# sebcossu/yocto_raytracing

Measured on AMD Instinct MI355X. Metric: Mrays/sec + ms/frame, instance10000 1920×1080×64spp, 1/2/4/8 MI355X, higher is better.
Workload: dtype f32; 1 GPU; instance10000 1920x1080 8x8 spp, amb 0.1, one frame per step; scene=instance10000, width=1920, height=1080, spp=64, parallelism=single GPU, algorithm=wavefront

## Files before the change

### yocto_raytracing_amd/csrc/packet_trace.h

```cpp
#pragma once

#include "descent_asm.h"
#include "fast_div.h"
#include "wide_asm.h"
#include "trace_common.h"

namespace yrt {

__device__ __forceinline__ int uniform(int x) { return __builtin_amdgcn_readfirstlane(x); }
__device__ __forceinline__ int lane_now() {
    int l;
    asm volatile("v_mbcnt_lo_u32_b32 %0, -1, 0\n v_mbcnt_hi_u32_b32 %0, -1, %0" : "=v"(l));
    return l;
}
__device__ __forceinline__ unsigned long long ballot(bool p) { return __ballot(p); }
extern "C" __device__ int yrt_llvm_writelane(int value, int lane, int old) __asm("llvm.amdgcn.writelane.i32");
__device__ __forceinline__ int writelane(int old, int value, int lane) { return yrt_llvm_writelane(value, lane, old); }

typedef int sgpr4 __attribute__((ext_vector_type(4)));
typedef int sgpr8 __attribute__((ext_vector_type(8)));
typedef int sgpr16 __attribute__((ext_vector_type(16)));
template <typename V>
__device__ __forceinline__ float4 rec_of(const V& v, int k) {
    return {__int_as_float(v[4 * k]), __int_as_float(v[4 * k + 1]), __int_as_float(v[4 * k + 2]),
// ... 629 lines not shown
                inst_next = lstart;
                inst_end = lstart + lcount;
                avail = lmask;
                if (LM) {
                    const uint32_t skip = (lcl >> 16) & 0x7fffu;
                    if (skip) {
                        const uint32_t keep = ~skip & ((1u << lcount) - 1u);
                        if (!keep) {
                            inst_end = inst_next;
                        } else {
                            inst_next = lstart + __builtin_ctz(keep);
                            inst_end = lstart + 32 - __builtin_clz(keep);
                        }
                    }
                }
                level = 1;
                base = sp;
            } else {
                const bool in = lane_in(lmask);
                unsigned long long leaf_hits = 0;
                DBG_CHECK(lstart >= 0 && lstart + lcount <= S.nsprims, 2, lstart, lcount, level, kind, sp);
#ifdef YRT_WIDE_STATS
                if (!COUNT) wc.box++, wc.prim += (unsigned)lcount;
#endif
                if (kind == kind_triangles) {
                    for (int i = lstart; i < lstart + lcount; i++) {
                        float4 pv[3];
                        ld_records_at<3>(S.sprims, (unsigned)(3 * i), pv);
                        if (COUNT && in) wc.prim++;
                        if (COUNT && (me & 1)) wc.wprim++;
                        float t, w1, w2;
                        const unsigned long long hm =
                            tri_hit_mask<true>(co, cd, tmin, tmax, xyz(pv[0]), xyz(pv[1]), xyz(pv[2]), t, w1, w2, lmask);
                        if (hm) {
                            const bool h = lane_in(hm);
                            tmax = h ? t : tmax;
                            hslot = h ? cur_slot : hslot;
                            hei = h ? ibits(pv[0].w) : hei;
                            hw1 = h ? w1 : hw1;
                            hw2 = h ? w2 : hw2;
                            leaf_hits |= hm;
                        }
                    }
                } else {
                    for (int i = lstart; i < lstart + lcount; i++) {
                        float4 pv[3];
                        ld_records_at<3>(S.sprims, (unsigned)(3 * i), pv);
                        if (COUNT && in) wc.prim++;
                        if (COUNT && (me & 1)) wc.wprim++;
                        float t;
                        vec4f ew;
                        const ray3 lr = {co, cd, tmin, tmax};
                        bool h = kind == kind_lines ? line_hit(lr, xyz(pv[0]), xyz(pv[1]), pv[1].w, pv[2].x, t, ew)
                                                    : point_hit(lr, xyz(pv[0]), pv[1].x, t, ew);
                        h = h && in;
                        tmax = h ? t : tmax;
                        hslot = h ? cur_slot : hslot;
                        hei = h ? ibits(pv[0].w) : hei;
                        hw1 = h ? ew.y : hw1;
                        hw2 = h ? ew.z : hw2;
                        leaf_hits |= ballot(h);
                    }
                }
                done |= leaf_hits & ballot(is_nan(tmax));
                avail &= ~done;
            }
        }
        bool finished = false;
        for (;;) {
            if (level == 1 && sp == base) {
                if (inst_next < inst_end) {
                    const int k = inst_next++;
                    DBG_CHECK(k >= 0 && k < S.ninst, 3, k, inst_end, sp, base, 0);
#ifdef YRT_WIDE_STATS
                    if (!COUNT) wc.inst++;
#endif
                    float4 fr[4];
                    ld_records_at<4>(S.tinst, (unsigned)(4 * k), fr);
                    const frame3f f = {xyz(fr[0]), xyz(fr[1]), xyz(fr[2]), xyz(fr[3])};
                    co = transform_point_inverse(f, wo);
                    const bool ident = (uniform(ibits(fr[0].w)) & (int)inst_identity_bit) != 0;
                    if (ident)
                        cd = icd, ci = ici;
                    else
                        enter_direction(f, wd, live & ~done, cd, ci);
                    const uint32_t rk = (uint32_t)uniform(ibits(fr[3].w));
                    pbase = S.spair + spine_record_f4 * (rk & 0x3fffffffu);
                    kind = (int)(rk >> 30);
                    cur_slot = k;
                    mask = avail;
                    if (COUNT && (mask & me)) wc.inst++;
                    node = 0;
                    oct = ident ? ioct : wave_octant(ci, live & ~done);
                    if (mask) break;
                    continue;
                }
                level = 0;
                avail = live & ~done;
                pbase = ptop;
                co = wo;
                cd = wd;
                {
                    const int t = wave * 64 + lane_now();
                    ci = {wi_lds[0][t], wi_lds[1][t], wi_lds[2][t]};
                }
                oct = woct;
            }
            if (sp == 0) {
                finished = true;
                break;
            }
            if constexpr (SM) {
                sp--;
                node = __builtin_amdgcn_readlane(stk_node, sp);
                mask = ((unsigned long long)(uint32_t)__builtin_amdgcn_readlane(stk_mhi, sp) << 32 |
                        (uint32_t)__builtin_amdgcn_readlane(stk_mlo, sp)) &
                       ~done;
                if (mask) break;
            } else {
                mask = avail;
                if (!mask) {
                    sp = level ? base : 0;
                    continue;
                }
                sp--;
                node = __builtin_amdgcn_readlane(stk_node, sp);
                break;
            }
        }
        if (finished) {
            if (!LM) break;
            lstep = true;
        }
    }
#ifdef YRT_WIDE_STATS
    if (!COUNT) {
        const unsigned long long hitl = ballot(hslot >= 0) & live;
        if ((threadIdx.x & 63) == 0) {
            unsigned long long* line = g_first_stats + 16 * ((blockIdx.x * 7u + threadIdx.x / 64u) & 1023u);
            const unsigned long long v[10] = {1, wc.tex, wc.wnode, wc.inst, wc.wprim, wc.box, wc.prim, 0,
                                              (unsigned long long)__popcll(live), (unsigned long long)__popcll(hitl)};
            for (int i = 0; i < 10; i++) atomicAdd(line + i, v[i]);
        }
        wc = work_counts{};
    }
#endif
    if (hslot < 0) return false;
    hr.slot = hslot;
    hr.ei = hei;
    hr.ew = {1 - hw1 - hw2, hw1, hw2, 0};
    hr.dist = tmax;
    return true;
}

__device__ __forceinline__ void ld_wide_record(const f4* wbase, uint32_t off, float4 (&r)[7]) {
    sgpr16 a;
    sgpr8 b;
    sgpr4 c;
    asm volatile(
        "s_load_dwordx16 %0, %3, %4\n s_load_dwordx8 %1, %3, %4 offset:0x40\n s_load_dwordx4 %2, %3, %4 offset:0x60\n"
        " s_waitcnt lgkmcnt(0)"
        : "=&s"(a), "=&s"(b), "=&s"(c)
        : "s"(wbase), "s"(uniform((int)off)));
#pragma unroll
    for (int k = 0; k < 4; k++) r[k] = rec_of(a, k);
    r[4] = rec_of(b, 0), r[5] = rec_of(b, 1), r[6] = rec_of(c, 0);
}

template <int OCT>
__device__ __forceinline__ void wide_tests(const float4 (&r)[7], vec3f co, vec3f ci, float tmin, float tmax,
                                           unsigned long long mask, uint32_t (&w)[4], unsigned long long (&m)[4]) {
    const float lx[4] = {r[0].x, r[0].y, r[0].z, r[0].w}, ly[4] = {r[1].x, r[1].y, r[1].z, r[1].w},
                lz[4] = {r[2].x, r[2].y, r[2].z, r[2].w}, hx[4] = {r[3].x, r[3].y, r[3].z, r[3].w},
                hy[4] = {r[4].x, r[4].y, r[4].z, r[4].w}, hz[4] = {r[5].x, r[5].y, r[5].z, r[5].w};
    w[0] = (uint32_t)uniform(ibits(r[6].x)), w[1] = (uint32_t)uniform(ibits(r[6].y));
    w[2] = (uint32_t)uniform(ibits(r[6].z)), w[3] = (uint32_t)uniform(ibits(r[6].w));
#pragma unroll
    for (int k = 0; k < 4; k++) {
        if (k < 2 || w[k] != wide_leaf) {
            m[k] = ballot(box_oct<OCT>(co, ci, tmin, tmax, lx[k], ly[k], lz[k], hx[k], hy[k], hz[k])) & mask;
        } else
            m[k] = 0;
    }
}

template <int OCT>
__device__ __forceinline__ bool wide_step(const float4 (&r)[7], vec3f co, vec3f ci, float tmin, float tmax,
                                          uint32_t& cur, unsigned long long& mask, int& sp, int& stk_word,
                                          int& stk_mlo, int& stk_mhi, int floor, unsigned long long done) {
    uint32_t w[4];
    unsigned long long m[4];
    wide_tests<OCT>(r, co, ci, tmin, tmax, mask, w, m);
    unsigned long long cm = 0;
    uint32_t cw = 0;
    {
        uint32_t ow;
        unsigned long long om;
        sp = uniform(sp);
        asm volatile(
            "s_cmp_lg_u64 %[m3], 0\n"
            "s_cbranch_scc1 .Lyb32_%=\n"
            "s_cmp_lg_u64 %[m2], 0\n"
            "s_cbranch_scc1 .Lyb21_%=\n"
            "s_cmp_lg_u64 %[m1], 0\n"
            "s_cbranch_scc1 .Lyb10_%=\n"
            "s_cmp_lg_u64 %[m0], 0\n"
            "s_cbranch_scc1 .Lyfin0_%=\n"
            "s_mov_b64 %[cm], 0\n"
            "s_mov_b32 %[cw], 0\n"
            "s_branch .Lyend_%=\n"
            ".Lyb32_%=:\n"
            "s_cmp_lg_u64 %[m2], 0\n"
            "s_cbranch_scc0 .Lyb31_%=\n"
            "s_mov_b32 m0, %[sp]\n"
            "v_writelane_b32 %[sw], %[w3], m0\n"
            "v_writelane_b32 %[sl], %[l3], m0\n"
            "v_writelane_b32 %[sh], %[h3], m0\n"
            "s_add_u32 %[sp], %[sp], 1\n"
            "s_branch .Lyb21_%=\n"
            ".Lyb31_%=:\n"
            "s_cmp_lg_u64 %[m1], 0\n"
            "s_cbranch_scc0 .Lyb30_%=\n"
            "s_mov_b32 m0, %[sp]\n"
            "v_writelane_b32 %[sw], %[w3], m0\n"
            "v_writelane_b32 %[sl], %[l3], m0\n"
            "v_writelane_b32 %[sh], %[h3], m0\n"
            "s_add_u32 %[sp], %[sp], 1\n"
            "s_branch .Lyb10_%=\n"
            ".Lyb30_%=:\n"
            "s_cmp_lg_u64 %[m0], 0\n"
            "s_cbranch_scc0 .Lyfin3_%=\n"
            "s_mov_b32 m0, %[sp]\n"
            "v_writelane_b32 %[sw], %[w3], m0\n"
            "v_writelane_b32 %[sl], %[l3], m0\n"
            "v_writelane_b32 %[sh], %[h3], m0\n"
            "s_add_u32 %[sp], %[sp], 1\n"
            "s_branch .Lyfin0_%=\n"
            ".Lyb21_%=:\n"
            "s_cmp_lg_u64 %[m1], 0\n"
            "s_cbranch_scc0 .Lyb20_%=\n"
            "s_mov_b32 m0, %[sp]\n"
            "v_writelane_b32 %[sw], %[w2], m0\n"
            "v_writelane_b32 %[sl], %[l2], m0\n"
            "v_writelane_b32 %[sh], %[h2], m0\n"
            "s_add_u32 %[sp], %[sp], 1\n"
            "s_branch .Lyb10_%=\n"
            ".Lyb20_%=:\n"
            "s_cmp_lg_u64 %[m0], 0\n"
            "s_cbranch_scc0 .Lyfin2_%=\n"
            "s_mov_b32 m0, %[sp]\n"
            "v_writelane_b32 %[sw], %[w2], m0\n"
            "v_writelane_b32 %[sl], %[l2], m0\n"
            "v_writelane_b32 %[sh], %[h2], m0\n"
            "s_add_u32 %[sp], %[sp], 1\n"
            "s_branch .Lyfin0_%=\n"
            ".Lyb10_%=:\n"
            "s_cmp_lg_u64 %[m0], 0\n"
            "s_cbranch_scc0 .Lyfin1_%=\n"
            "s_mov_b32 m0, %[sp]\n"
            "v_writelane_b32 %[sw], %[w1], m0\n"
            "v_writelane_b32 %[sl], %[l1], m0\n"
            "v_writelane_b32 %[sh], %[h1], m0\n"
            "s_add_u32 %[sp], %[sp], 1\n"
            "s_branch .Lyfin0_%=\n"
            ".Lyfin3_%=:\n"
            "s_mov_b32 %[cw], %[w3]\n"
            "s_mov_b64 %[cm], %[m3]\n"
            "s_branch .Lyend_%=\n"
            ".Lyfin2_%=:\n"
            "s_mov_b32 %[cw], %[w2]\n"
            "s_mov_b64 %[cm], %[m2]\n"
            "s_branch .Lyend_%=\n"
            ".Lyfin1_%=:\n"
            "s_mov_b32 %[cw], %[w1]\n"
            "s_mov_b64 %[cm], %[m1]\n"
            "s_branch .Lyend_%=\n"
            ".Lyfin0_%=:\n"
            "s_mov_b32 %[cw], %[w0]\n"
            "s_mov_b64 %[cm], %[m0]\n"
            ".Lyend_%=:\n"
            : [cw] "=&s"(ow), [cm] "=&s"(om), [sp] "+s"(sp), [sw] "+v"(stk_word), [sl] "+v"(stk_mlo),
              [sh] "+v"(stk_mhi)
            : [w0] "s"(w[0]), [w1] "s"(w[1]), [w2] "s"(w[2]), [w3] "s"(w[3]), [m0] "s"(m[0]), [m1] "s"(m[1]),
              [m2] "s"(m[2]), [m3] "s"(m[3]), [l0] "s"((uint32_t)m[0]), [l1] "s"((uint32_t)m[1]),
              [l2] "s"((uint32_t)m[2]), [l3] "s"((uint32_t)m[3]), [h0] "s"((uint32_t)(m[0] >> 32)),
              [h1] "s"((uint32_t)(m[1] >> 32)), [h2] "s"((uint32_t)(m[2] >> 32)), [h3] "s"((uint32_t)(m[3] >> 32))
            : "m0", "scc");
        sp = uniform(sp);
        cw = (uint32_t)uniform((int)ow);
        cm = (unsigned long long)(uint32_t)uniform((int)(om >> 32)) << 32 | (uint32_t)uniform((int)(uint32_t)om);
    }
    mask = cm;
    cur = cw;
    if (cm) return !(cw & wide_leaf);
    {
        int n = 0;
        if (inner_pop(floor, done, n, mask, sp, stk_word, stk_mlo, stk_mhi)) {
            cur = (uint32_t)n;
            return !(cur & wide_leaf);
        }
    }
    return false;
}

template <int OCT, int LDSN, bool ASM = false>
__device__ __forceinline__ void wide_descend(const f4* base, const float4* lds, vec3f co, vec3f ci,
// ... 203 lines not shown
```

### yocto_raytracing_amd/csrc/wavefront.hip

```cpp
#include <hip/hip_runtime.h>

#include <algorithm>
#include <cstdio>
#include <cstdlib>
#include <cstring>
#include <stdexcept>
#include <type_traits>

#include "item_magic.h"
#include "packet_trace.h"
#include "trace_common.h"
#include "yrt_render.h"

namespace yrt {
namespace {

constexpr int WF_BLOCK = 256;
#ifndef YRT_PRIMARY_BLOCK
#define YRT_PRIMARY_BLOCK 64
#endif
#ifndef YRT_SHADOW_BLOCK
#define YRT_SHADOW_BLOCK 64
#endif
template <bool PACKET>
// ... 238 lines not shown
template <bool ANY, bool COUNT, bool PACKET, typename SE>
__device__ __forceinline__ tracer<ANY, COUNT, PACKET, SE> make_tracer(traversal_lds<PACKET, SE>& L) {
    tracer<ANY, COUNT, PACKET, SE> t;
    if constexpr (PACKET)
        t.lane_stk = nullptr;
    else
        t.lane_stk = L.lane + threadIdx.x;
    return t;
}

template <unsigned C>
__device__ __forceinline__ unsigned xcd_runs(unsigned b, unsigned n) {
    constexpr unsigned G = 8u * C;
    if (b >= n / G * G) return b;
    const unsigned w = b % G;
    return b - w + (w % 8u) * C + w / 8u;
}

#ifndef YRT_SHADOW_LIGHT_MINOR
#define YRT_SHADOW_LIGHT_MINOR 24
#endif
#ifndef YRT_XCD_CHUNK_PRIMARY
#define YRT_XCD_CHUNK_PRIMARY 256
#endif

__device__ __forceinline__ vec3f div3(vec3f ke, float rr) {
    if (!__ballot(!(div_nr_ok(ke.x, rr) && div_nr_ok(ke.y, rr) && div_nr_ok(ke.z, rr)))) {
        const float y = rcp_nr(rr);
        return {div_nr(ke.x, rr, y), div_nr(ke.y, rr, y), div_nr(ke.z, rr, y)};
    }
    return ke / rr;
}

__device__ __forceinline__ bool light_term_zero(int info, vec3f nrm, vec3f p, vec3f ro, vec3f l, float r, vec3f ke) {
    const int cls = (info >> 26) & 15;
    const float sd = smax(0.0f, dot(nrm, l));
    const bool first = info >= 0 && cls != 0 && (info & 3) != kind_lines && sd == 0.0f;
    if (!ballot(first)) return false;
    vec3f v, h, ker;
    float vlen, hlen;
    normalize_len(ro - p, v, vlen);
    normalize_len(v + l, h, hlen);
    ker = div3(ke, r * r);
    const float x = smax(0.0f, dot(nrm, h));
    const bool ker_ok = fabsf(ker.x) < 0x1p100f && fabsf(ker.y) < 0x1p100f && fabsf(ker.z) < 0x1p100f;
    const bool ls_zero =
        cls == 1 ? x >= 0.0f && x <= 1.0f
                 : x == 0.0f || (x >= 0x1p-126f && x < 1.0f &&
                                 (float)(16 << ((cls - 2) & 15)) * __builtin_amdgcn_logf(x) < -151.0f);
    return first && ker_ok && ls_zero;
}

__device__ __forceinline__ ray3 camera_ray_w(const dev_camera& cam, int W, int H, int ns, int i, int j, int ii,
                                             int jj, bool in_range = false) {
    const float fns = (float)ns, fw = (float)W, fh = (float)H;
    const float a = ii + 0.5f, b = jj + 0.5f;
    float u, v;
    if (in_range || !__ballot(!(div_nr_ok(a, fns) && div_nr_ok(b, fns)))) {
        const float y = rcp_nr(fns);
        u = i + div_nr(a, fns, y), v = j + div_nr(b, fns, y);
    } else {
        u = i + a / fns, v = j + b / fns;
    }
    if (in_range || !__ballot(!(div_nr_ok(u, fw) && div_nr_ok(v, fh)))) {
        u = div_nr(u, fw, rcp_nr(fw)), v = div_nr(v, fh, rcp_nr(fh));
    } else {
        u = u / fw, v = v / fh;
    }
    vec3f q;
    q.x = cam.ox + (u - 0.5f) * cam.w * cam.xx + (v - 0.5f) * cam.h * cam.yx - cam.focus * cam.zx;
    q.y = cam.oy + (u - 0.5f) * cam.w * cam.xy + (v - 0.5f) * cam.h * cam.yy - cam.focus * cam.zy;
    q.z = cam.oz + (u - 0.5f) * cam.w * cam.xz + (v - 0.5f) * cam.h * cam.yz - cam.focus * cam.zz;
    const vec3f o = {cam.ox, cam.oy, cam.oz};
    vec3f d;
    float len;
    normalize_len(q - o, d, len);
    return {o, d, ray_eps, flt_max};
}

#ifndef YRT_BUNDLE_ITEMS
#define YRT_BUNDLE_ITEMS 64
#endif
constexpr int bundle_g = YRT_BUNDLE_ITEMS;
static_assert(bundle_g >= 1 && bundle_g <= 64, "one item per lane of k_bundle_lists");
#ifndef YRT_BUNDLE_MIN_TOP
#define YRT_BUNDLE_MIN_TOP 8
#endif
#ifndef YRT_LISTS_MIN_SPP
#define YRT_LISTS_MIN_SPP 9
#endif
constexpr int bundle_max = 16;
constexpr int bundle_recs = 5;
constexpr int bundle_max_lights = 8;
#ifndef YRT_CAMERA_LIST_MAX
#define YRT_CAMERA_LIST_MAX 32
#endif
constexpr int camera_list_max = YRT_CAMERA_LIST_MAX;

template <int CTRL, int ROWS>
__device__ __forceinline__ int dpp_i(int v) {
    return __builtin_amdgcn_mov_dpp(v, CTRL, ROWS, 0xf, false);
}
__device__ __forceinline__ int fkey(int b) { return b ^ ((b >> 31) & 0x7fffffff); }
template <bool MAX>
__device__ __forceinline__ float wave_fold(float f) {
    auto op = [](int a, int b) { return MAX ? max(a, b) : min(a, b); };
    int v = fkey(__float_as_int(f));
    v = op(v, dpp_i<0x121, 0xf>(v));
    v = op(v, dpp_i<0x122, 0xf>(v));
    v = op(v, dpp_i<0x124, 0xf>(v));
    v = op(v, dpp_i<0x128, 0xf>(v));
    v = op(v, dpp_i<0x142, 0xa>(v));
    v = op(v, dpp_i<0x143, 0xc>(v));
    return __int_as_float(fkey(__builtin_amdgcn_readlane(v, 63)));
}
__device__ __forceinline__ float wave_fmin(float v) { return wave_fold<false>(v); }
__device__ __forceinline__ float wave_fmax(float v) { return wave_fold<true>(v); }
__device__ __forceinline__ void wave_box(float (&lo)[3], float (&hi)[3]) {
    int v[6];
    for (int a = 0; a < 3; a++) v[a] = fkey(__float_as_int(lo[a])), v[3 + a] = fkey(__float_as_int(hi[a]));
#define YRT_BOX_STEP(CTRL, ROWS)                                                  \
    {                                                                             \
        int t[6];                                                                 \
        for (int a = 0; a < 6; a++) t[a] = dpp_i<CTRL, ROWS>(v[a]);               \
        for (int a = 0; a < 6; a++) v[a] = a < 3 ? min(v[a], t[a]) : max(v[a], t[a]); \
    }
    YRT_BOX_STEP(0x121, 0xf)
    YRT_BOX_STEP(0x122, 0xf)
    YRT_BOX_STEP(0x124, 0xf)
    YRT_BOX_STEP(0x128, 0xf)
    YRT_BOX_STEP(0x142, 0xa)
    YRT_BOX_STEP(0x143, 0xc)
#undef YRT_BOX_STEP
    for (int a = 0; a < 3; a++) {
        lo[a] = __int_as_float(fkey(__builtin_amdgcn_readlane(v[a], 63)));
        hi[a] = __int_as_float(fkey(__builtin_amdgcn_readlane(v[3 + a], 63)));
    }
}

__device__ __forceinline__ void store_item_box(const wf_buffers& B, int idx, bool has_p, vec3f p) {
    const bool fin = has_p && __builtin_isfinite(p.x) && __builtin_isfinite(p.y) && __builtin_isfinite(p.z);
    const bool bad = has_p && !fin;
    float lo[3] = {fin ? p.x : INFINITY, fin ? p.y : INFINITY, fin ? p.z : INFINITY};
    float hi[3] = {fin ? p.x : -INFINITY, fin ? p.y : -INFINITY, fin ? p.z : -INFINITY};
    wave_box(lo, hi);
    const bool any_bad = ballot(bad) != 0;
    if ((threadIdx.x & 63) == 0) {
        const int item = idx >> 6;
        gstore(B.pbox, 2 * item, lo[0], lo[1], lo[2], any_bad ? -1.0f : 0.0f);
        gstore(B.pbox, 2 * item + 1, hi[0], hi[1], hi[2], 0.0f);
    }
}

template <bool COUNT, bool PACKET, typename SE, int BS = packet_block, int LDSN = 0, bool LIST = false>
__device__ __forceinline__ bool primary_samples(const dev_scene_view& S, const dev_render_args& A, const chunk_args& C,
                                                const wf_buffers& B, tracer<false, COUNT, PACKET, SE, BS>& T, int idx,
                                                work_counts& wc, const float4* lds = nullptr) {
    const int nsamp = C.npix * C.spp;
    bool valid = false;
    ray3 ray = {{0, 0, 0}, {0, 0, 1}, ray_eps, flt_max};
    const bool magic = YRT_ITEM_MAGIC && uniform(C.M.on) != 0;
    int list_tile = -1;
    if (magic) {
        const bool in_range = uniform(C.M.div_ok) != 0;
        const int ns = A.samples;
        int lx, ly, i, j, ii, jj;
        if (uniform(C.M.pow2)) {
            const uint32_t item = (uint32_t)uniform(idx) >> 6;
            const uint32_t sl = (uint32_t)uniform(C.M.spp_log2), lane = (uint32_t)idx & 63u;
            const uint32_t ct = item >> sl;
            const uint32_t t = (uint32_t)uniform((int)(uint32_t)(C.pix0 >> 6)) + ct;
            const tile_magic G = {(uint32_t)uniform((int)C.M.tiles_x.mul), (uint32_t)uniform((int)C.M.tiles_x.shift),
                                  (uint32_t)uniform((int)C.M.tiles_x.d),  (uint32_t)uniform((int)C.M.band.mul),
                                  (uint32_t)uniform((int)C.M.band.shift), (uint32_t)uniform((int)C.M.band.d)};
            const uint32_t w0 = (item & ((1u << sl) - 1u)) << (6u - sl);
            if (sl == 6u)
                valid = pixel_of_tile(A, G, t, w0, lx, ly, i, j);
            else
                valid = pixel_of_tile(A, G, t, w0 + (lane >> sl), lx, ly, i, j);
            const uint32_t q = lane & ((1u << sl) - 1u), nl = sl >> 1;
            ii = (int)(q & ((1u << nl) - 1u)), jj = (int)(q >> nl);
            valid = valid && idx < nsamp;
            if ((int)(item * 64u) < nsamp) list_tile = (int)ct;
        } else {
            const uint32_t pl = magic_div((uint32_t)idx, C.M.spp), q = (uint32_t)idx - pl * (uint32_t)C.spp;
            const uint32_t p = (uint32_t)C.pix0 + pl;
            valid = idx < nsamp && pixel_of_tile(A, tile_magic_of(C), p / (TILE * TILE), p % (TILE * TILE), lx, ly, i, j);
            jj = (int)magic_div(q, C.M.samples), ii = (int)q - jj * ns;
        }
        if (valid)
            ray = camera_ray_w(A.cam, A.width, A.height, ns, i, j, ii, jj, in_range);
        else if (idx < nsamp)
            store_not_sample(B, idx);
    } else if (idx < nsamp) {
        const long long p = C.pix0 + idx / C.spp;
        const int q = idx % C.spp;
        int lx, ly, i, j;
        valid = pixel_of(A, C.tiles_x, p, lx, ly, i, j);
        if (valid) {
            const int ns = A.samples;
            ray = camera_ray_w(A.cam, A.width, A.height, ns, i, j, q % ns, q / ns);
        } else {
            store_not_sample(B, idx);
        }
    }
    hit_record hr = {-1, -1, {0, 0, 0, 0}, 0};
    bool hit;
    if constexpr (PACKET) {
        const f4* lbase = nullptr;
        int ln = -1;
        if (LIST && !COUNT) {
            const int nsamp = C.npix * C.spp;
            const int i0 = uniform(idx) & ~63, i1 = min(i0 + 63, nsamp - 1);
            int t0, t1;
            if (magic && list_tile >= 0) {
                t0 = t1 = list_tile;
            } else if (magic) {
                const uint32_t mul = (uint32_t)uniform((int)C.M.spp.mul), sh = (uint32_t)uniform((int)C.M.spp.shift);
                t0 = (int)(magic_div((uint32_t)i0, mul, sh) / (TILE * TILE));
                t1 = (int)(magic_div((uint32_t)max(i1, 0), mul, sh) / (TILE * TILE));
            } else {
                t0 = i0 / C.spp / (TILE * TILE), t1 = i1 / C.spp / (TILE * TILE);
            }
            const bool zero_dir = valid && ray.d.x == 0.0f && ray.d.y == 0.0f && ray.d.z == 0.0f;
            if (t0 == t1 && i0 < nsamp && !ballot(zero_dir)) {
                ln = uniform(B.ccount[t0]);
                lbase = B.clist + (size_t)t0 * camera_list_max * 2;
            }
        }
        hit = packet_first<COUNT, BS, true, LDSN, LIST>(S, ray, valid, hr, wc, B.trel, lds, lbase, ln);
    } else {
        hit = T.trace(S, ray, valid, hr, wc);
    }
    vec3f hp = {0, 0, 0};
    if (valid) {
        if (COUNT && hit) wc.hits++;
        hp = store_hit_surface(S, B, idx, hit, hr);
    }
    if (!COUNT && B.bundles) store_item_box(B, idx, valid && hit, hp);
    return valid;
}


__global__ __launch_bounds__(WF_BLOCK) void k_chunk_setup(const f4* __restrict__ tpair, int nrec, float ox, float oy,
                                                          float oz, f4* __restrict__ trel, unsigned* queue,
                                                          unsigned long long* lstats, int* count, int count_ints,
                                                          unsigned long long* counters, int counter_words) {
    const int i = blockIdx.x * WF_BLOCK + threadIdx.x;
    const int stride = gridDim.x * WF_BLOCK;
    if (tpair)
        for (int k = i; k < nrec; k += stride) {
            const float4 r = ld4(tpair + k);
            trel[k] = {r.x - ox, r.y - oy, r.z - oz, r.w};
        }
    if (i < 32) queue[i] = 0u;
    if (lstats && i < list_sums) lstats[i] = 0ull;
    for (int k = i; k < count_ints; k += stride) count[k] = 0;
    if (counters)
        for (int k = i; k < counter_words; k += stride) counters[k] = 0ull;
}

#ifndef YRT_SHARED_TAIL
#define YRT_SHARED_TAIL 32
#endif
constexpr unsigned tail_flag = 0x80000000u;
constexpr unsigned gcd_u(unsigned a, unsigned b) { return b ? gcd_u(b, a % b) : a; }
template <unsigned RUN, unsigned CS>
__device__ __forceinline__ unsigned head_items(unsigned n_items) {
    constexpr unsigned G = 8u * (RUN / gcd_u(RUN, CS) * CS);
    return YRT_SHARED_TAIL ? (n_items - n_items / YRT_SHARED_TAIL) / G * G : 0u;
}
template <unsigned CS>
__device__ __forceinline__ unsigned chunk_fetch(unsigned* counter, unsigned* gcounter, unsigned limit) {
    const unsigned k = __hip_atomic_fetch_add(counter, 1u, __ATOMIC_RELAXED, __HIP_MEMORY_SCOPE_AGENT);
    if (!YRT_SHARED_TAIL || k * CS + CS <= limit) return k * CS;
    return tail_flag | __hip_atomic_fetch_add(gcounter, 1u, __ATOMIC_RELAXED, __HIP_MEMORY_SCOPE_AGENT) * CS;
}

struct chunk_ring {
    static constexpr unsigned R = 4;
    unsigned base[R], tag[R], reads[R], taken;
};

template <unsigned CS>
__device__ __forceinline__ void chunk_ring_init(chunk_ring& ring, unsigned* counter, unsigned* gcounter = nullptr,
                                                unsigned limit = ~0u) {
    static_assert(CS >= 2, "a chunk's middle slot fetches the next chunk");
    if (threadIdx.x < chunk_ring::R) {
        ring.tag[threadIdx.x] = threadIdx.x == 0 ? 0u : ~0u;
        ring.reads[threadIdx.x] = threadIdx.x == 0 ? 0u : CS;
    }
    if (threadIdx.x == 0) {
        ring.base[0] = chunk_fetch<CS>(counter, gcounter, limit);
        ring.taken = 0;
    }
    __syncthreads();
}

template <unsigned CS>
__device__ __forceinline__ unsigned chunk_ring_next(chunk_ring& ring, unsigned* counter, unsigned lane,
                                                    unsigned* gcounter = nullptr, unsigned limit = ~0u) {
    constexpr unsigned R = chunk_ring::R;
    unsigned t = 0;
    if (lane == 0) t = __hip_atomic_fetch_add(&ring.taken, 1u, __ATOMIC_RELAXED, __HIP_MEMORY_SCOPE_WORKGROUP);
    t = (unsigned)__builtin_amdgcn_readfirstlane((int)t);
    const unsigned g = t / CS, o = t % CS;
    if (o == CS / 2) {
        const unsigned e1 = (g + 1) % R;
        unsigned nbase = 0;
        if (lane == 0) nbase = chunk_fetch<CS>(counter, gcounter, limit);
        nbase = (unsigned)__builtin_amdgcn_readfirstlane((int)nbase);
        while (__hip_atomic_load(&ring.reads[e1], __ATOMIC_ACQUIRE, __HIP_MEMORY_SCOPE_WORKGROUP) != CS)
            __builtin_amdgcn_s_sleep(1);
        if (lane == 0) {
            ring.base[e1] = nbase;
            __hip_atomic_store(&ring.reads[e1], 0u, __ATOMIC_RELAXED, __HIP_MEMORY_SCOPE_WORKGROUP);
            __hip_atomic_store(&ring.tag[e1], g + 1, __ATOMIC_RELEASE, __HIP_MEMORY_SCOPE_WORKGROUP);
        }
    }
    const unsigned e = g % R;
    while (__hip_atomic_load(&ring.tag[e], __ATOMIC_ACQUIRE, __HIP_MEMORY_SCOPE_WORKGROUP) != g)
        __builtin_amdgcn_s_sleep(1);
    const unsigned q = (unsigned)__builtin_amdgcn_readfirstlane((int)ring.base[e]) + o;
    if (lane == 0) __hip_atomic_fetch_add(&ring.reads[e], 1u, __ATOMIC_RELEASE, __HIP_MEMORY_SCOPE_WORKGROUP);
    return q;
}

template <unsigned RUN>
__device__ __forceinline__ unsigned xcd_item(unsigned q, unsigned xcd, unsigned n_items) {
    const unsigned full = n_items / (8u * RUN) * (8u * RUN);
    const unsigned per_xcd = full / 8u;
    return q < per_xcd ? ((q / RUN) * 8u + xcd) * RUN + q % RUN : full + (q - per_xcd) * 8u + xcd;
}
template <unsigned RUN>
__device__ __forceinline__ unsigned split_item(unsigned q, unsigned xcd, unsigned n_items, unsigned head) {
    if (!YRT_SHARED_TAIL) return xcd_item<RUN>(q, xcd, n_items);
    if (q & tail_flag) return head + (q & ~tail_flag);
    return ((q / RUN) * 8u + xcd) * RUN + q % RUN;
}

#ifdef YRT_TAIL_STATS
static __device__ unsigned long long g_tail[2][8192][4];
__device__ __forceinline__ void tail_record(int k, unsigned long long t0, unsigned items) {
    const unsigned gw = blockIdx.x * (blockDim.x / 64u) + threadIdx.x / 64u;
    if ((threadIdx.x & 63) == 0 && gw < 8192u) {
        unsigned long long* e = g_tail[k][gw];
        e[0] = t0, e[1] = __builtin_amdgcn_s_memrealtime(), e[2] = items, e[3] = blockIdx.x % 8u;
    }
}
#endif

template <bool COUNT, bool PACKET, typename SE, bool LIST = false>
__global__ __launch_bounds__(YRT_PRIMARY_BLOCK, YRT_TRACE_WAVES) void k_primary(dev_scene_view S, dev_render_args A,
                                                               chunk_args C, wf_buffers B,
                                                               unsigned long long* counters) {
    constexpr int BS = YRT_PRIMARY_BLOCK;
    __shared__ traversal_lds<PACKET, SE> lds;
    auto T = make_tracer<false, COUNT, PACKET, SE>(lds);
    const int idx = (int)xcd_runs<YRT_XCD_CHUNK_PRIMARY>(blockIdx.x, gridDim.x) * BS + threadIdx.x;
    work_counts wc;
    const bool valid = primary_samples<COUNT, PACKET, SE, packet_block, 0, LIST>(S, A, C, B, T, idx, wc);
    flush_block<2, BS>(counters, {cnt_rays, cnt_samples}, {valid ? 1ull : 0ull, valid ? 1ull : 0ull});
    if (COUNT) flush_work(counters, wc);
}

constexpr int SP_BLOCK = 1024;
#ifndef YRT_PRIMARY_WAVES
#define YRT_PRIMARY_WAVES YRT_TRACE_WAVES
#endif
#ifndef YRT_PRIMARY_SP_BLOCK
#define YRT_PRIMARY_SP_BLOCK \
    (YRT_PRIMARY_WAVES == 7 ? 448 : YRT_PRIMARY_WAVES == 6 ? 768 : YRT_PRIMARY_WAVES == 5 ? 640 : SP_BLOCK)
#endif
static_assert((YRT_PRIMARY_WAVES * 4 * 64) % YRT_PRIMARY_SP_BLOCK == 0, "whole blocks per CU");
#ifndef YRT_PRIMARY_LDS_RECORDS
#define YRT_PRIMARY_LDS_RECORDS 511
#endif
#ifndef YRT_PRIMARY_PERSIST_MIN_ITEMS
#define YRT_PRIMARY_PERSIST_MIN_ITEMS 0
#endif
#ifndef YRT_PRIMARY_BLOCK_CHUNK
#define YRT_PRIMARY_BLOCK_CHUNK 16
#endif
template <typename SE, int LDSN, bool LIST = false>
__global__ __launch_bounds__(YRT_PRIMARY_SP_BLOCK, YRT_PRIMARY_WAVES) void k_primary_persist(dev_scene_view S,
                                                                                dev_render_args A, chunk_args C,
                                                                                wf_buffers B,
                                                                                unsigned long long* counters) {
    constexpr unsigned CS = YRT_PRIMARY_BLOCK_CHUNK;
    constexpr int SPB = YRT_PRIMARY_SP_BLOCK;
    __shared__ chunk_ring ring;
    __shared__ dev_render_args A_lds;
    __shared__ chunk_args C_lds;
    __shared__ wf_buffers B_lds;
    __shared__ float4 lds_rec[LDSN > 0 ? LDSN * spine_record_f4 : 1];
    if constexpr (LDSN > 0) {
        const int n = min(LDSN, S.ntnodes) * spine_record_f4;
        const float4* src = reinterpret_cast<const float4*>(B.trel);
        for (int i = (int)threadIdx.x; i < n; i += SPB) lds_rec[i] = src[i];
    }
    if (threadIdx.x == 0) A_lds = A, C_lds = C, B_lds = B;
    const unsigned lane = threadIdx.x & 63;
    const unsigned xcd = blockIdx.x % 8u;
    unsigned* counter = B.queue + 16 + xcd;
    unsigned* gcounter = B.queue + 24;
    const unsigned n_items = (unsigned)((C.npix * C.spp + 63) / 64);
    const unsigned head = head_items<YRT_XCD_CHUNK_PRIMARY, CS>(n_items);
    chunk_ring_init<CS>(ring, counter, gcounter, head / 8u);
    tracer<false, false, true, SE, SPB> T;
    T.lane_stk = nullptr;
    work_counts wc;
    unsigned valid_n = 0;
#ifdef YRT_TAIL_STATS
    const unsigned long long tail_t0 = __builtin_amdgcn_s_memrealtime();
    unsigned tail_items = 0;
#endif
    for (;;) {
        const unsigned q = chunk_ring_next<CS>(ring, counter, lane, gcounter, head / 8u);
        const unsigned it = split_item<YRT_XCD_CHUNK_PRIMARY>(q, xcd, n_items, head);
        if (it >= n_items) break;
#ifdef YRT_TAIL_STATS
        tail_items++;
#endif
        asm volatile("" ::: "memory");
        const bool valid = primary_samples<false, true, SE, SPB, LDSN, LIST>(S, A_lds, C_lds, B_lds, T,
                                                                            (int)(it * 64) + lane_now(), wc, lds_rec);
        valid_n += (unsigned)__popcll(ballot(valid));
    }
#ifdef YRT_TAIL_STATS
    tail_record(0, tail_t0, tail_items);
#endif
    const unsigned long long mine = lane == 0 ? (unsigned long long)valid_n : 0ull;
    flush_block<2, SPB>(counters, {cnt_rays, cnt_samples}, {mine, mine});
}

__device__ __forceinline__ vec3f ray_origin(const wf_buffers& B, int idx) {
    const float* r = B.rays + (size_t)idx * 8;
    return {r[0], r[1], r[2]};
}

template <bool PACKET, typename SE>
__global__ __launch_bounds__(WF_BLOCK, YRT_TRACE_WAVES) void k_rays_first(dev_scene_view S, int n, wf_buffers B,
                                                                          unsigned long long* counters) {
    __shared__ traversal_lds<PACKET, SE> lds;
    auto T = make_tracer<false, false, PACKET, SE>(lds);
    work_counts wc;
    const int idx = blockIdx.x * WF_BLOCK + threadIdx.x;
    const bool valid = idx < n;
    ray3 ray = {{0, 0, 0}, {0, 0, 1}, ray_eps, flt_max};
    if (valid) {
        const float* r = B.rays + (size_t)idx * 8;
        ray = {{r[0], r[1], r[2]}, {r[3], r[4], r[5]}, r[6], r[7]};
    }
    hit_record hr = {-1, -1, {0, 0, 0, 0}, 0};
    const bool hit = T.trace(S, ray, valid, hr, wc);
    if (valid) store_hit_surface(S, B, idx, hit, hr);
    flush_block<2>(counters, {cnt_rays, cnt_samples}, {valid ? 1ull : 0ull, valid ? 1ull : 0ull});
}

template <bool COUNT, bool PACKET, typename SE>
__global__ __launch_bounds__(WF_BLOCK, YRT_TRACE_WAVES) void k_bounce(dev_scene_view S, int level, wf_buffers B,
                                                     unsigned long long* counters) {
    __shared__ traversal_lds<PACKET, SE> lds;
    auto T = make_tracer<false, COUNT, PACKET, SE>(lds);
    work_counts wc;
    unsigned long long rays = 0;
    const int stride = gridDim.x * WF_BLOCK;
    for (int g = 0; g < level_segments; g++) {
    const int n = *seg_counter(B.count, level, g);
    const int nround = (n + stride - 1) / stride;
    for (int round = 0; round < nround; round++) {
        const int j = round * stride + blockIdx.x * WF_BLOCK + threadIdx.x;
        const bool valid = j < n;
        const int idx = g * B.seg + j;
        ray3 ray = {{0, 0, 0}, {0, 0, 1}, ray_eps, flt_max};
        if (valid) {
            float4 o = ld4(B.ray_o(level) + idx), d = ld4(B.ray_d(level) + idx);
            ray = {xyz(o), xyz(d), ray_eps, flt_max};
            rays++;
        }
        hit_record hr = {-1, -1, {0, 0, 0, 0}, 0};
        const bool hit = T.trace(S, ray, valid, hr, wc);
        if (valid) {
            if (COUNT && hit) wc.hits++;
            store_hit_surface(S, B, idx, hit, hr);
        }
    }
    }
    flush_block<1>(counters, {cnt_rays}, {rays});
    if (COUNT) flush_work(counters, wc);
}

template <bool COUNT, bool PACKET, typename SE, bool WIDE>
__global__ __launch_bounds__(shadow_block<PACKET>(), YRT_SHADOW_WAVES) void k_shadow(dev_scene_view S, int level,
                                                                     int nsamp_level0, wf_buffers B,
                                                                     unsigned long long* counters, float4 cam4) {
    const vec3f cam_o = xyz(cam4);
    constexpr int BS = shadow_block<PACKET>();
    __shared__ traversal_lds<PACKET, SE> lds;
    auto T = make_tracer<true, COUNT, PACKET, SE>(lds);
    const unsigned lin = level ? blockIdx.x
                               : xcd_runs<YRT_SHADOW_LIGHT_MINOR>(blockIdx.y * gridDim.x + blockIdx.x,
                                                                  gridDim.x * gridDim.y);
    const int li = level ? (int)blockIdx.y : (int)(lin % gridDim.y);
    const int bx = level ? (int)blockIdx.x : (int)(lin / gridDim.y);
    const f4* lr = S.lights + 6 * li;
    const frame3f lf = {xyz(ld4(lr)), xyz(ld4(lr + 1)), xyz(ld4(lr + 2)), xyz(ld4(lr + 3))};
    const vec3f lp0 = xyz(ld4(lr + 4)), ke = xyz(ld4(lr + 5));
    work_counts wc;
    unsigned long long rays = 0, culled = 0;
    const int stride = gridDim.x * BS;
    for (int g = 0; g < (level ? level_segments : 1); g++) {
    const int n = level ? *seg_counter(B.count, level, g) : nsamp_level0;
    const int nround = (n + stride - 1) / stride;
    for (int round = 0; round < nround; round++) {
        const int j = round * stride + bx * BS + threadIdx.x;
        const int idx = g * B.seg + j;
        bool valid = false;
        int info = -1;
        float r = 1.0f;
        float4 s1 = {0, 0, 0, 0}, ro4 = make_float4(cam_o.x, cam_o.y, cam_o.z, 0.0f);
        ray3 sr = {{0, 0, 0}, {0, 0, 1}, 0.01f, 1.0f};
        constexpr bool CULL = !COUNT;
        if (j < n) {
            float4 s0 = ld4s(B.surf0 + idx);
            if (CULL) {
                s1 = ld4s(B.surf1 + idx);
                if (level) ro4 = ld4(B.ray_o(level) + idx);
            }
            info = sample_state(s0);
            if (info >= 0) {
                const vec3f p = xyz(s0);
                vec3f tp = transform_point(lf, lp0 - p);
                vec3f l;
                normalize_len(tp, l, r);
                sr = {p, l, 0.01f, r - 0.01f};
                valid = true;
                rays++;
            }
        }
        if (CULL) {
            if (light_term_zero(info, xyz(s1), sr.o, xyz(ro4), sr.d, r, ke)) {
                stb(B.occl + (size_t)li * B.capacity + idx, 1);
                valid = false;
                culled++;
            }
        }
        hit_record hr;
        bool occ;
        if constexpr (WIDE)
            occ = packet_occluded_wide2(S, sr, valid);
        else
            occ = T.trace(S, sr, valid, hr, wc);
        if (valid) stb(B.occl + (size_t)li * B.capacity + idx, occ ? 1 : 0);
    }
    }
    flush_block<2, BS>(counters, {cnt_shadow_rays, cnt_shadow_culled}, {rays, culled});
    if (COUNT) {
        flush_work(counters, wc);
        flush(counters, cnt_shadow_box_tests, wc.box);
        flush(counters, cnt_shadow_inst_entries, wc.inst);
        flush(counters, cnt_shadow_prim_tests, wc.prim);
        flush(counters, cnt_shadow_wave_node_visits, wc.wnode);
    }
}

template <bool PACKET, typename SE, bool WIDE>
__global__ __launch_bounds__(shadow_block<PACKET>(), YRT_SHADOW_WAVES) void k_rays_shadow(dev_scene_view S, int nsamp,
                                                                                          wf_buffers B,
                                                                                          unsigned long long* counters) {
    constexpr int BS = shadow_block<PACKET>();
    __shared__ traversal_lds<PACKET, SE> lds;
    auto T = make_tracer<true, false, PACKET, SE>(lds);
    const unsigned lin = xcd_runs<YRT_SHADOW_LIGHT_MINOR>(blockIdx.y * gridDim.x + blockIdx.x, gridDim.x * gridDim.y);
    const int li = (int)(lin % gridDim.y);
    const int idx = (int)(lin / gridDim.y) * BS + (int)threadIdx.x;
    const f4* lr = S.lights + 6 * li;
    const frame3f lf = {xyz(ld4(lr)), xyz(ld4(lr + 1)), xyz(ld4(lr + 2)), xyz(ld4(lr + 3))};
// ... 2202 lines not shown
```

Before: 31450 Mrays/s.

## Add nested list-driven primary traversal with octant-specialized descent for camera tiles

Adds a specialized primary-ray traversal that walks the per-tile camera candidate list, descends the top-level spine and then each instance's bottom-level spine. Octant-templated descent is selected through a switch, and list state and inverse directions are kept in LDS to save registers. It is enabled by default when the list path is used without LDS record caching. This aims to cut divergence and redundant node tests in the generic packet traversal, at the cost of more code size and LDS use, and a risk of register pressure from the eight-way dispatch.

After: 32790 Mrays/s, median of 6. +4.3%, better.

```diff
diff --git a/yocto_raytracing_amd/csrc/packet_trace.h b/yocto_raytracing_amd/csrc/packet_trace.h
--- a/yocto_raytracing_amd/csrc/packet_trace.h
+++ b/yocto_raytracing_amd/csrc/packet_trace.h
@@ -805,6 +805,260 @@
     hr.dist = tmax;
     return true;
 }
+
+#if !defined(YRT_FIRST_NESTED)
+#define YRT_FIRST_NESTED 1
+#endif
+#define YRT_OCT_DISPATCH(oct, X) \
+    switch (oct) {               \
+        case 0: X(0); break;     \
+        case 1: X(1); break;     \
+        case 2: X(2); break;     \
+        case 3: X(3); break;     \
+        case 4: X(4); break;     \
+        case 5: X(5); break;     \
+        case 6: X(6); break;     \
+        case 7: X(7); break;     \
+        default: X(8); break;    \
+    }
+template <int BS = packet_block>
+__device__ __forceinline__ bool packet_first_list(const dev_scene_view& S, const ray3& wray, bool valid,
+                                                  hit_record& hr, work_counts& wc, const f4* trel, const f4* lbase,
+                                                  int ln) {
+    static_assert(spine_len == 2, "packet_first_list walks two-node spine records");
+    constexpr bool SM = YRT_STACK_MASKS;
+    const unsigned long long live = ballot(valid && !is_nan(wray.tmin) && !is_nan(wray.tmax));
+    if (!live) return false;
+    const int fl = __builtin_ctzll(live);
+    const vec3f wo = {__int_as_float(__builtin_amdgcn_readlane(__float_as_int(wray.o.x), fl)),
+                      __int_as_float(__builtin_amdgcn_readlane(__float_as_int(wray.o.y), fl)),
+                      __int_as_float(__builtin_amdgcn_readlane(__float_as_int(wray.o.z), fl))};
+    const vec3f wd = wray.d;
+    float tmin = wray.tmin, tmax = wray.tmax;
+    asm volatile("" : "+v"(tmin), "+v"(tmax));
+    vec3f co = wo, cd = wd, ci = rcp3(wd, live);
+    __shared__ float wi_lds[3][BS];
+    {
+        const int t = (int)threadIdx.x;
+        wi_lds[0][t] = ci.x, wi_lds[1][t] = ci.y, wi_lds[2][t] = ci.z;
+    }
+    float hw1 = 0, hw2 = 0;
+    int hslot = -1, hei = -1;
+    int stk_node = 0, stk_mlo = 0, stk_mhi = 0;
+    unsigned long long alive = live, mask = 0;
+    int sp = 0, node = 0;
+    const int woct = wave_octant(ci, live);
+    vec3f icd, ici;
+    enter_direction(frame3f{{1, 0, 0}, {0, 1, 0}, {0, 0, 1}, {0, 0, 0}}, wd, live, icd, ici);
+    const int ioct = wave_octant(ici, live);
+    __shared__ int list_lds[BS / 64][4];
+    int* const lst = list_lds[threadIdx.x >> 6];
+    lst[0] = (int)(unsigned)(unsigned long long)lbase, lst[1] = (int)((unsigned long long)lbase >> 32);
+    lst[2] = ln, lst[3] = 0;
+    for (;;) {
+        uint32_t lcl = 0;
+        mask = 0;
+        asm volatile("" ::: "memory");
+        const int lend = uniform(lst[2]);
+        int lnext = uniform(lst[3]);
+        if (lend < 0) {
+            if (lnext == 0) node = 0, mask = alive, lnext = 1;
+        } else {
+            const f4* lb = (const f4*)((unsigned long long)(unsigned)uniform(lst[1]) << 32 | (unsigned)uniform(lst[0]));
+            while (lnext < lend) {
+                float4 e[2];
+                ld_records_at<2>(lb, (unsigned)(2 * lnext), e);
+                lnext++;
+#ifdef YRT_WIDE_STATS
+                wc.tex++;
+#endif
+                const unsigned long long lanes = alive;
+                unsigned long long m;
+#define YRT_LE(o) m = list_entry_test<o>(ci, tmin, tmax, e, lanes)
+                YRT_OCT_DISPATCH(woct, YRT_LE)
+#undef YRT_LE
+                if (m) {
+                    const int w0 = uniform(ibits(e[0].w));
+                    const uint32_t w1 = (uint32_t)uniform(ibits(e[1].w));
+                    mask = m;
+                    if (w1 & leaf_bit) {
+                        node = w0, lcl = w1;
+                    } else {
+                        stk_node = writelane(stk_node, w0, sp);
+                        if constexpr (SM) {
+                            stk_mlo = writelane(stk_mlo, (int)(uint32_t)m, sp);
+                            stk_mhi = writelane(stk_mhi, (int)(uint32_t)(m >> 32), sp);
+                        }
+                        sp++;
+                        node = w0 + spine_record_bytes;
+                    }
+                    break;
+                }
+            }
+        }
+        if (!mask) break;
+        lst[3] = lnext;
+        asm volatile("" ::: "memory");
+        for (;;) {
+            if (!(lcl & leaf_bit)) {
+                DBG_CHECK(node >= 0 && (node % spine_record_bytes) == 0 && sp >= 0 && sp < 63 &&
+                              node / spine_record_bytes < S.ntnodes,
+                          1, node, sp, 0, 0, 0);
+                const unsigned long long pop_arg = SM ? ~alive : alive;
+#define YRT_FD(o)                                                                                            \
+    first_descend<o, false, true, 0, SM, true>(trel, co, ci, tmin, tmax, 0ull, node, mask, sp, stk_node, stk_mlo, \
+                                               stk_mhi, lcl, wc, 0, pop_arg, nullptr)
+                YRT_OCT_DISPATCH(woct, YRT_FD)
+#undef YRT_FD
+            }
+            if (mask) {
+                unsigned long long avail = mask;
+                const int lstart = node, lcount = (int)(lcl & 0xffffu);
+                int inst_next = lstart, inst_end = lstart + lcount;
+                const uint32_t skip = (lcl >> 16) & 0x7fffu;
+                if (skip) {
+                    const uint32_t keep = ~skip & ((1u << lcount) - 1u);
+                    if (!keep) {
+                        inst_end = inst_next;
+                    } else {
+                        inst_next = lstart + __builtin_ctz(keep);
+                        inst_end = lstart + 32 - __builtin_clz(keep);
+                    }
+                }
+                const int base = sp;
+                for (int k = inst_next; k < inst_end && avail; k++) {
+                    DBG_CHECK(k >= 0 && k < S.ninst, 3, k, inst_end, sp, base, 0);
+#ifdef YRT_WIDE_STATS
+                    wc.inst++;
+#endif
+                    float4 fr[4];
+                    ld_records_at<4>(S.tinst, (unsigned)(4 * k), fr);
+                    const frame3f f = {xyz(fr[0]), xyz(fr[1]), xyz(fr[2]), xyz(fr[3])};
+                    co = transform_point_inverse(f, wo);
+                    const bool ident = (uniform(ibits(fr[0].w)) & (int)inst_identity_bit) != 0;
+                    if (ident)
+                        cd = icd, ci = ici;
+                    else
+                        enter_direction(f, wd, alive, cd, ci);
+                    const uint32_t rk = (uint32_t)uniform(ibits(fr[3].w));
+                    unsigned long long sbits = (unsigned long long)(S.spair + spine_record_f4 * (rk & 0x3fffffffu));
+                    sbits = (unsigned long long)(uint32_t)uniform((int)(sbits >> 32)) << 32 |
+                            (uint32_t)uniform((int)(uint32_t)sbits);
+                    asm volatile("" : "+s"(sbits));
+                    const f4* const sbase = (const f4*)sbits;
+                    const int kind = (int)(rk >> 30);
+                    const int soct = ident ? ioct : wave_octant(ci, alive);
+                    node = 0;
+                    mask = avail;
+                    for (;;) {
+                        DBG_CHECK(node >= 0 && (node % spine_record_bytes) == 0 && sp >= 0 && sp < 63 &&
+                                      (int)((sbase - S.spair) / 4) + node / spine_record_bytes < S.nsnodes,
+                                  1, node, sp, 1, (int)((sbase - S.spair) / 4), base);
+                        const unsigned long long pop_arg = SM ? ~alive : avail;
+#define YRT_FD(o)                                                                                              \
+    first_descend<o, false, false, 0, SM, true>(sbase, co, ci, tmin, tmax, 0ull, node, mask, sp, stk_node, stk_mlo, \
+                                                stk_mhi, lcl, wc, base, pop_arg, nullptr)
+                        YRT_OCT_DISPATCH(soct, YRT_FD)
+#undef YRT_FD
+                        if (mask) {
+                            const unsigned long long lmask = mask;
+                            const int pstart = node, pcount = (int)(lcl & 0xffffu);
+                            unsigned long long leaf_hits = 0;
+                            DBG_CHECK(pstart >= 0 && pstart + pcount <= S.nsprims, 2, pstart, pcount, 1, kind, sp);
+#ifdef YRT_WIDE_STATS
+                            wc.box++, wc.prim += (unsigned)pcount;
+#endif
+                            if (kind == kind_triangles) {
+                                for (int i = pstart; i < pstart + pcount; i++) {
+                                    float4 pv[3];
+                                    ld_records_at<3>(S.sprims, (unsigned)(3 * i), pv);
+                                    float t, w1, w2;
+                                    const unsigned long long hm = tri_hit_mask<true>(
+                                        co, cd, tmin, tmax, xyz(pv[0]), xyz(pv[1]), xyz(pv[2]), t, w1, w2, lmask);
+                                    if (hm) {
+                                        const bool h = lane_in(hm);
+                                        tmax = h ? t : tmax;
+                                        hslot = h ? k : hslot;
+                                        hei = h ? ibits(pv[0].w) : hei;
+                                        hw1 = h ? w1 : hw1;
+                                        hw2 = h ? w2 : hw2;
+                                        leaf_hits |= hm;
+                                    }
+                                }
+                            } else {
+                                const bool in = lane_in(lmask);
+                                for (int i = pstart; i < pstart + pcount; i++) {
+                                    float4 pv[3];
+                                    ld_records_at<3>(S.sprims, (unsigned)(3 * i), pv);
+                                    float t;
+                                    vec4f ew;
+                                    const ray3 lr = {co, cd, tmin, tmax};
+                                    bool h = kind == kind_lines
+                                                 ? line_hit(lr, xyz(pv[0]), xyz(pv[1]), pv[1].w, pv[2].x, t, ew)
+                                                 : point_hit(lr, xyz(pv[0]), pv[1].x, t, ew);
+                                    h = h && in;
+                                    tmax = h ? t : tmax;
+                                    hslot = h ? k : hslot;
+                                    hei = h ? ibits(pv[0].w) : hei;
+                                    hw1 = h ? ew.y : hw1;
+                                    hw2 = h ? ew.z : hw2;
+                                    leaf_hits |= ballot(h);
+                                }
+                            }
+                            const unsigned long long out = leaf_hits & ballot(is_nan(tmax));
+                            alive &= ~out;
+                            avail &= ~out;
+                        }
+                        if constexpr (SM) {
+                            if (!inner_pop(base, ~alive, node, mask, sp, stk_node, stk_mlo, stk_mhi)) break;
+                        } else {
+                            if (!avail) {
+                                sp = base;
+                                break;
+                            }
+                            if (!inner_pop_avail(base, avail, node, mask, sp, stk_node)) break;
+                        }
+                    }
+                }
+                co = wo;
+                cd = wd;
+                {
+                    const int t = (int)threadIdx.x;
+                    ci = {wi_lds[0][t], wi_lds[1][t], wi_lds[2][t]};
+                }
+            }
+            lcl = 0;
+            if constexpr (SM) {
+                if (!inner_pop(0, ~alive, node, mask, sp, stk_node, stk_mlo, stk_mhi)) break;
+            } else {
+                if (!alive) {
+                    sp = 0;
+                    break;
+                }
+                if (!inner_pop_avail(0, alive, node, mask, sp, stk_node)) break;
+            }
+        }
+    }
+#ifdef YRT_WIDE_STATS
+    {
+        const unsigned long long hitl = ballot(hslot >= 0) & live;
+        if ((threadIdx.x & 63) == 0) {
+            unsigned long long* line = g_first_stats + 16 * ((blockIdx.x * 7u + threadIdx.x / 64u) & 1023u);
+            const unsigned long long v[10] = {1, wc.tex, wc.wnode, wc.inst, wc.wprim, wc.box, wc.prim, 0,
+                                              (unsigned long long)__popcll(live), (unsigned long long)__popcll(hitl)};
+            for (int i = 0; i < 10; i++) atomicAdd(line + i, v[i]);
+        }
+        wc = work_counts{};
+    }
+#endif
+    if (hslot < 0) return false;
+    hr.slot = hslot;
+    hr.ei = hei;
+    hr.ew = {1 - hw1 - hw2, hw1, hw2, 0};
+    hr.dist = tmax;
+    return true;
+}
+#undef YRT_OCT_DISPATCH
 
 __device__ __forceinline__ void ld_wide_record(const f4* wbase, uint32_t off, float4 (&r)[7]) {
     sgpr16 a;
diff --git a/yocto_raytracing_amd/csrc/wavefront.hip b/yocto_raytracing_amd/csrc/wavefront.hip
--- a/yocto_raytracing_amd/csrc/wavefront.hip
+++ b/yocto_raytracing_amd/csrc/wavefront.hip
@@ -414,7 +414,8 @@
     }
 }
 
-template <bool COUNT, bool PACKET, typename SE, int BS = packet_block, int LDSN = 0, bool LIST = false>
+template <bool COUNT, bool PACKET, typename SE, int BS = packet_block, int LDSN = 0, bool LIST = false,
+          bool NESTED = false>
 __device__ __forceinline__ bool primary_samples(const dev_scene_view& S, const dev_render_args& A, const chunk_args& C,
                                                 const wf_buffers& B, tracer<false, COUNT, PACKET, SE, BS>& T, int idx,
                                                 work_counts& wc, const float4* lds = nullptr) {
@@ -490,7 +491,10 @@
                 lbase = B.clist + (size_t)t0 * camera_list_max * 2;
             }
         }
-        hit = packet_first<COUNT, BS, true, LDSN, LIST>(S, ray, valid, hr, wc, B.trel, lds, lbase, ln);
+        if constexpr (NESTED && LIST && !COUNT && LDSN == 0)
+            hit = packet_first_list<BS>(S, ray, valid, hr, wc, B.trel, lbase, ln);
+        else
+            hit = packet_first<COUNT, BS, true, LDSN, LIST>(S, ray, valid, hr, wc, B.trel, lds, lbase, ln);
     } else {
         hit = T.trace(S, ray, valid, hr, wc);
     }
@@ -685,7 +689,7 @@
         tail_items++;
 #endif
         asm volatile("" ::: "memory");
-        const bool valid = primary_samples<false, true, SE, SPB, LDSN, LIST>(S, A_lds, C_lds, B_lds, T,
+        const bool valid = primary_samples<false, true, SE, SPB, LDSN, LIST, YRT_FIRST_NESTED != 0>(S, A_lds, C_lds, B_lds, T,
                                                                             (int)(it * 64) + lane_now(), wc, lds_rec);
         valid_n += (unsigned)__popcll(ballot(valid));
     }
```
